# Angtian/VoGE

Hardware: AMD Instinct MI355X
Metric: forward+backward frames/sec at 512^2, 50k Gaussians; ray-trace HBM GB/s vs peak (higher is better)
Workload: dtype f32; 1 GPU; cfg3_50k_512: 50000 random Gaussians (scalar sigmas), 512x512, K=40, max_point_per_bin=-1, fwd+bwd (grads to verts, sigmas, colors); launch=hip graph replay, 4 consecutive steps per graph launch, parallelism=1 gpu

## Files before the change

include/voge_hip.h:

```cpp
#ifndef VOGE_HIP_H
#define VOGE_HIP_H

#include <stddef.h>
#include <stdint.h>

#ifdef __cplusplus
extern "C" {
#endif

#define VOGE_ABI_VERSION 7

#define VOGE_ERR_BAD_ARG (-1)
#define VOGE_ERR_WORKSPACE (-2)
#define VOGE_ERR_K_TOO_LARGE (-3)

#define VOGE_MAX_K 256

typedef void *voge_stream_t;

int voge_abi_version(void);

const char *voge_error_string(int code);

size_t voge_trace_workspace_bytes(int B, int N, int H, int W);
// ... 19 lines not shown
                   const float *g_dsd, int P, long nrows, int W, int K, void *workspace,
                   size_t workspace_bytes, float *g_ray, float *g_mus, float *g_isg,
                   voge_stream_t stream);

size_t voge_trace_bwd_workspace_bytes(int P);

int voge_trace_topk_fwd_iso(const float *mus, const float *a, const float *rays,
                            const float *cam_fwd, const float *cones, int B, int N, int H, int W, int K,
                            float thr_act, void *workspace, size_t workspace_bytes,
                            int32_t *idx, float *len, float *act, float *dsd, int32_t *cnt,
                            voge_stream_t stream);
int voge_trace_bwd_iso(const float *mus, const float *a, const float *rays, const int32_t *idx,
                       const int32_t *cnt, const float *g_len, const float *g_act, const float *g_dsd,
                       int P, long nrows, int W, int K, void *workspace, size_t workspace_bytes,
                       float *g_ray, float *g_mus, float *g_a, voge_stream_t stream);
size_t voge_trace_bwd_iso_workspace_bytes(int P);

int voge_trace_topk_fwd_iso_view(const float *verts, const float *sigmas, const float *origin, int shared,
                                 int sigma_mode, const float *rays, const float *cam_fwd, const float *cones,
                                 int B, int N, int H, int W, int K, float thr_act, void *workspace,
                                 size_t workspace_bytes, int32_t *idx, float *len, float *act, float *dsd,
                                 int32_t *cnt, voge_stream_t stream);
int voge_trace_bwd_iso_view(const float *verts, const float *sigmas, const float *origin, int shared,
                            int sigma_mode, const float *rays, const int32_t *idx, const int32_t *cnt,
                            const float *g_len, const float *g_act, const float *g_dsd, int B, int N, long nrows,
                            int W, int K, void *workspace, size_t workspace_bytes, float *g_ray,
                            float *g_verts, float *g_sigmas, voge_stream_t stream);

int voge_bin_gaussians(const float *points, const int64_t *cloud_to_packed_first_idx,
                       const int64_t *num_points_per_cloud, int B, int P, int H, int W, const float *radius,
                       int bin_size, int max_points_per_bin, int32_t *bin_elems, voge_stream_t stream);

int voge_trace_lean_fwd(const float *mus, const float *isigmas, const float *rays, const float *cam_fwd,
                        const float *cones, int B, int N, int H, int W, int K, float thr_act, void *workspace,
                        size_t workspace_bytes, int32_t *idx, float *len, int32_t *cnt, float *records,
                        voge_stream_t stream);
int voge_fragments_fwd(const float *mus, const float *isigmas, const float *rays, const float *cam_fwd,
                       const float *cones, int B, int N, int H, int W, int K, float thr_act, float occ,
                       void *workspace, size_t workspace_bytes, int32_t *idx, float *len, float *act, float *dsd,
                       int32_t *cnt, float *weight, int64_t *valid_num, voge_stream_t stream);
int voge_fragments_fwd_iso(const float *mus, const float *a, const float *rays, const float *cam_fwd,
                           const float *cones, int B, int N, int H, int W, int K, float thr_act, float occ,
                           void *workspace, size_t workspace_bytes, int32_t *idx, float *len, float *act,
                           float *dsd, int32_t *cnt, float *weight, int64_t *valid_num, float *records,
                           voge_stream_t stream);
int voge_fragments_fwd_iso_view(const float *verts, const float *sigmas, const float *origin, int shared,
                                int sigma_mode, const float *rays, const float *cam_fwd, const float *cones,
                                int B, int N, int H, int W, int K, float thr_act, float occ, void *workspace,
                                size_t workspace_bytes, int32_t *idx, float *len, float *act, float *dsd,
                                int32_t *cnt, float *weight, int64_t *valid_num, float *records, voge_stream_t stream);

size_t voge_fragment_bwd_workspace_bytes(int P);
int voge_fragment_act_dsd_iso(const float *records, const float *rays, const int32_t *idx, const float *len,
                              const int32_t *cnt, long npix, int K, int P, float *act, float *dsd, voge_stream_t stream);
int voge_composite_fwd_iso(const int32_t *idx, const int32_t *cnt, const float *len, const float *records,
                           const float *rays, float occ, long npix, int K, float *weight, int64_t *valid_num,
                           voge_stream_t stream);
int voge_composite_shade_fwd_iso(int32_t *idx, const int32_t *cnt, const float *len, const float *records,
                                 const float *rays, float occ, const float *colors, const float *bg, float thr,
                                 long npix, int K, int C, long Nattr, float *weight, int64_t *valid_num, float *rgb,
                                 float *img, float *wsum, voge_stream_t stream);
int voge_composite_fwd_rec(int32_t *idx, const int32_t *cnt, const float *len, const float *records, const float *rays,
                           float occ, long npix, int K, float *weight, int64_t *valid_num, float *act, float *dsd,
                           voge_stream_t stream);
int voge_composite_shade_fwd_rec(int32_t *idx, const int32_t *cnt, const float *len, const float *records,
                                 const float *rays, float occ, const float *colors, const float *bg, float thr,
                                 long npix, int K, int C, long Nattr, float *weight, int64_t *valid_num, float *rgb,
                                 float *img, float *wsum, float *act, float *dsd, voge_stream_t stream);
int voge_fragment_shade_bwd(const float *mus, const float *isigmas, const float *rays, const float *colors,
                            const int32_t *idx, const int32_t *cnt, const float *weight, const float *act,
                            const float *len, const float *dsd, const float *rgb, const float *wsum, const float *bg,
                            float thr, const float *g_img, long g_stride_pix, long g_stride_c, float occ, int P,
                            long nrows, int W, int K, int C, long Nattr, void *workspace, size_t workspace_bytes,
                            float *g_mus, float *g_isigmas, float *g_colors, voge_stream_t stream);
int voge_fragment_shade_bwd_iso(const float *records, const float *sigmas, int shared, int sigma_mode,
                                const float *rays, const float *colors, const int32_t *idx, const int32_t *cnt,
                                const float *weight, const float *act, const float *len, const float *dsd,
                                const float *rgb, const float *wsum, const float *bg, float thr,
                                const float *g_img, long g_stride_pix, long g_stride_c, float occ, int B, int N,
                                long nrows, int W, int K, int C, long Nattr, void *workspace, size_t workspace_bytes, float *g_verts,
                                float *g_sigmas, float *g_colors, voge_stream_t stream);

size_t voge_frame_bwd_acc_bytes(int P);
int voge_frame_trace_fwd_iso(const float *verts, const float *sigmas, int shared, int sigma_mode, const float *R,
                             const float *T, const float *focal, const float *pp, int row0, int stripe_h, int pitch,
                             int behind, int B, int N, int h, int W, int K, float thr_act, void *workspace,
                             size_t workspace_bytes, int32_t *idx, float *len, int32_t *cnt, float *records,
                             float *rays, float *origin, voge_stream_t stream);
int voge_frame_shade_fwd_iso(int32_t *idx, const int32_t *cnt, const float *len, const float *records,
                             const float *rays, float occ, const float *colors, const float *bg, float thr,
                             long npix, int K, int C, long Nattr, float *weight, int64_t *valid_num,
                             float *rgb, float *img, float *wsum, float *sil, void *bwd_acc, size_t bwd_acc_bytes,
                             voge_stream_t stream);
int voge_frame_shade_bwd_iso(const float *records, const float *sigmas, int shared, int sigma_mode,
                             const float *rays, const float *colors, const int32_t *idx, const int32_t *cnt,
                             const float *weight, const float *len, const float *rgb, const float *wsum,
                             const float *bg, float thr, const float *g_img, long g_stride_pix, long g_stride_c,
                             float occ, int B, int N, long nrows, int W, int K, int C, long Nattr, void *acc_zeroed,
                             size_t acc_bytes, float *g_verts, float *g_sigmas, float *g_colors, voge_stream_t stream);
int voge_frame_merge_bwd_iso(const float *records, const float *sigmas, int shared, int sigma_mode,
                             const float *rays, const float *attr, const int32_t *idx, const int32_t *cnt,
                             const float *weight, const float *len, const float *g_rgb, long g_stride_pix,
                             long g_stride_c, const float *g_wsum, const float *wsum_fwd, float occ, int B, int N, long nrows,
                             int W, int K, int C, long Nattr, void *acc_zeroed, size_t acc_bytes, float *g_verts,
                             float *g_sigmas, float *g_attr, voge_stream_t stream);

size_t voge_frame_bwd_gen_acc_bytes(int P);
int voge_frame_trace_fwd_gen(const float *verts, const float *sigmas, int shared_verts, int shared_sigmas, int kind,
                             const float *R, const float *T, const float *focal, const float *pp, int row0, int stripe_h,
                             int pitch, int behind, int B, int N, int h, int W, int K, float thr_act, void *workspace,
                             size_t workspace_bytes, int32_t *idx, float *len, int32_t *cnt, float *records, float *rays,
                             float *origin, voge_stream_t stream);
int voge_frame_shade_fwd_rec(int kind, int32_t *idx, const int32_t *cnt, const float *len, const float *records,
                             const float *rays, float occ, const float *colors, const float *bg, float thr,
                             long npix, int K, int C, long Nattr, float *weight, int64_t *valid_num,
                             float *rgb, float *img, float *wsum, float *sil, float *act, float *dsd, void *bwd_acc,
                             size_t bwd_acc_bytes, voge_stream_t stream);
int voge_frame_bwd_gen(int form, const float *records, int shared_verts, int shared_sigmas, int kind, const float *rays,
                       const float *attr, const int32_t *idx, const int32_t *cnt, const float *weight, const float *act,
                       const float *len, const float *dsd, const float *rgb, const float *wsum, const float *bg, float thr,
                       const float *g, long g_stride0, long g_stride1, const float *g_hitlen, float occ, int B, int N,
                       long nrows, int W, int K, int C, long Nattr, void *acc, size_t acc_bytes, int acc_is_zero,
                       float *g_verts, float *g_sigmas, float *g_attr, voge_stream_t stream);

int voge_frame_trace_fwd_ori(const float *verts, const float *scales, const float *quats, int shared_verts, int shared_sigmas,
                             int sigma_mode, const float *R, const float *T, const float *focal, const float *pp, int row0,
                             int stripe_h, int pitch, int behind, int B, int N, int h, int W, int K, float thr_act, void *workspace,
                             size_t workspace_bytes, int32_t *idx, float *len, int32_t *cnt, float *records, float *rays,
                             float *origin, voge_stream_t stream);
int voge_frame_bwd_ori(int form, const float *records, const float *scales, const float *quats, int shared_verts, int shared_sigmas,
                       int sigma_mode, const float *rays, const float *attr, const int32_t *idx, const int32_t *cnt,
                       const float *weight, const float *act, const float *len, const float *dsd, const float *rgb, const float *wsum,
                       const float *bg, float thr, const float *g, long g_stride0, long g_stride1, const float *g_hitlen, float occ,
                       int B, int N, long nrows, int W, int K, int C, long Nattr, void *acc, size_t acc_bytes, int acc_is_zero,
                       float *g_verts, float *g_scales, float *g_quats, float *g_attr, voge_stream_t stream);

int voge_fragment_merge_bwd(const float *mus, const float *isigmas, const float *rays, const float *attr,
                            const int32_t *idx, const int32_t *cnt, const float *weight, const float *act,
                            const float *len, const float *dsd, const float *g_rgb, long g_stride_pix,
                            long g_stride_c, const float *g_wsum, float occ, int P, long nrows, int W, int K, int C,
                            long Nattr, void *workspace, size_t workspace_bytes, float *g_mus, float *g_isigmas,
                            float *g_attr, voge_stream_t stream);
int voge_fragment_merge_bwd_iso(const float *records, const float *sigmas, int shared, int sigma_mode,
                                const float *rays, const float *attr, const int32_t *idx, const int32_t *cnt,
                                const float *weight, const float *act, const float *len, const float *dsd,
                                const float *g_rgb, long g_stride_pix, long g_stride_c, const float *g_wsum,
                                float occ, int B, int N, long nrows, int W, int K, int C, long Nattr,
                                void *workspace, size_t workspace_bytes, float *g_verts, float *g_sigmas,
                                float *g_attr, voge_stream_t stream);

int voge_fragment_bwd_iso(const float *records, const float *sigmas, int shared, int sigma_mode, const float *rays,
                          const int32_t *idx, const int32_t *cnt, const float *weight, const float *act,
                          const float *len, const float *dsd, const float *g_weight, long gw_stride_pix,
                          long gw_stride_k, const float *g_hitlen, float occ, int B, int N, long nrows, int W, int K,
                          void *workspace, size_t workspace_bytes, float *g_verts, float *g_sigmas,
                          voge_stream_t stream);
int voge_fragment_bwd(const float *mus, const float *isigmas, const float *rays, const int32_t *idx,
                      const int32_t *cnt, const float *weight, const float *act, const float *len,
                      const float *dsd, const float *g_weight, long gw_stride_pix, long gw_stride_k,
                      const float *g_hitlen, float occ, int P, long nrows, int W, int K, void *workspace,
                      size_t workspace_bytes, float *g_mus, float *g_isigmas, voge_stream_t stream);

int voge_composite_fwd(const int32_t *idx, const int32_t *cnt, const float *act, const float *len,
                       const float *dsd, float occ, long npix, int K, float *weight,
                       int64_t *valid_num, voge_stream_t stream);

// ... 91 lines not shown
```

voge_amd/_lib.py:

```python
import ctypes
import os

_HERE = os.path.dirname(os.path.abspath(__file__))
LIB_PATH = os.environ.get("VOGE_HIP_LIB") or os.path.join(_HERE, "libvoge_hip.so")
ABI_VERSION = 7
MAX_K = 256

_c_void_p = ctypes.c_void_p
_c_int = ctypes.c_int
_c_long = ctypes.c_long
_c_float = ctypes.c_float
_c_size_t = ctypes.c_size_t

SIGNATURES = {
    "voge_abi_version": (_c_int, []),
    "voge_error_string": (ctypes.c_char_p, [_c_int]),
    "voge_trace_workspace_bytes": (_c_size_t, [_c_int] * 4),
    "voge_trace_pool_usage": (_c_int, [_c_void_p, _c_size_t] + [_c_int] * 4 + [_c_void_p] * 2),
    "voge_trace_topk_fwd": (_c_int, [_c_void_p] * 5 + [_c_int] * 5 + [_c_float, _c_void_p, _c_size_t]
                            + [_c_void_p] * 6),
    "voge_trace_topk_list_fwd": (_c_int, [_c_void_p] * 4 + [_c_int] * 9 + [_c_float] + [_c_void_p] * 6),
    "voge_trace_bwd": (_c_int, [_c_void_p] * 8 + [_c_int, _c_long, _c_int, _c_int, _c_void_p, _c_size_t] + [_c_void_p] * 4),
    "voge_trace_bwd_workspace_bytes": (_c_size_t, [_c_int]),
    "voge_trace_topk_fwd_iso": (_c_int, [_c_void_p] * 5 + [_c_int] * 5 + [_c_float, _c_void_p, _c_size_t]
                                + [_c_void_p] * 6),
    "voge_trace_bwd_iso": (_c_int, [_c_void_p] * 8 + [_c_int, _c_long, _c_int, _c_int, _c_void_p, _c_size_t] + [_c_void_p] * 4),
    "voge_trace_bwd_iso_workspace_bytes": (_c_size_t, [_c_int]),
    "voge_trace_topk_fwd_iso_view": (_c_int, [_c_void_p] * 3 + [_c_int] * 2 + [_c_void_p] * 3 + [_c_int] * 5
                                     + [_c_float, _c_void_p, _c_size_t] + [_c_void_p] * 6),
    "voge_trace_bwd_iso_view": (_c_int, [_c_void_p] * 3 + [_c_int] * 2 + [_c_void_p] * 6
                                + [_c_int, _c_int, _c_long, _c_int, _c_int, _c_void_p, _c_size_t] + [_c_void_p] * 4),
    "voge_bin_gaussians": (_c_int, [_c_void_p] * 3 + [_c_int] * 4 + [_c_void_p] + [_c_int] * 2 + [_c_void_p] * 2),
    "voge_fragments_fwd": (_c_int, [_c_void_p] * 5 + [_c_int] * 5 + [_c_float, _c_float, _c_void_p, _c_size_t] + [_c_void_p] * 8),
    "voge_fragments_fwd_iso": (_c_int, [_c_void_p] * 5 + [_c_int] * 5 + [_c_float, _c_float, _c_void_p, _c_size_t] + [_c_void_p] * 9),
    "voge_fragments_fwd_iso_view": (_c_int, [_c_void_p] * 3 + [_c_int] * 2 + [_c_void_p] * 3 + [_c_int] * 5
                                    + [_c_float, _c_float, _c_void_p, _c_size_t] + [_c_void_p] * 9),
    "voge_frame_trace_fwd_iso": (_c_int, [_c_void_p] * 2 + [_c_int] * 2 + [_c_void_p] * 4 + [_c_int] * 9
                                 + [_c_float, _c_void_p, _c_size_t] + [_c_void_p] * 7),
    "voge_frame_shade_fwd_iso": (_c_int, [_c_void_p] * 5 + [_c_float, _c_void_p, _c_void_p, _c_float, _c_long, _c_int, _c_int, _c_long]
                                 + [_c_void_p] * 7 + [_c_size_t, _c_void_p]),
    "voge_frame_shade_bwd_iso": (_c_int, [_c_void_p] * 2 + [_c_int] * 2 + [_c_void_p] * 9 + [_c_float, _c_void_p, _c_long, _c_long, _c_float]
                                 + [_c_int, _c_int, _c_long, _c_int, _c_int, _c_int, _c_long, _c_void_p, _c_size_t] + [_c_void_p] * 4),
    "voge_frame_merge_bwd_iso": (_c_int, [_c_void_p] * 2 + [_c_int] * 2 + [_c_void_p] * 7 + [_c_long, _c_long, _c_void_p, _c_void_p, _c_float]
                                 + [_c_int, _c_int, _c_long, _c_int, _c_int, _c_int, _c_long, _c_void_p, _c_size_t] + [_c_void_p] * 4),
    "voge_frame_bwd_acc_bytes": (_c_size_t, [_c_int]),
    "voge_frame_bwd_gen_acc_bytes": (_c_size_t, [_c_int]),
    "voge_frame_trace_fwd_gen": (_c_int, [_c_void_p] * 2 + [_c_int] * 3 + [_c_void_p] * 4 + [_c_int] * 9
                                 + [_c_float, _c_void_p, _c_size_t] + [_c_void_p] * 7),
    "voge_frame_shade_fwd_rec": (_c_int, [_c_int] + [_c_void_p] * 5 + [_c_float, _c_void_p, _c_void_p, _c_float, _c_long, _c_int, _c_int, _c_long]
                                 + [_c_void_p] * 9 + [_c_size_t, _c_void_p]),
    "voge_frame_bwd_gen": (_c_int, [_c_int, _c_void_p] + [_c_int] * 3 + [_c_void_p] * 11 + [_c_float, _c_void_p, _c_long, _c_long, _c_void_p, _c_float]
                           + [_c_int, _c_int, _c_long, _c_int, _c_int, _c_int, _c_long, _c_void_p, _c_size_t, _c_int] + [_c_void_p] * 4),
    "voge_frame_trace_fwd_ori": (_c_int, [_c_void_p] * 3 + [_c_int] * 3 + [_c_void_p] * 4 + [_c_int] * 9
                                 + [_c_float, _c_void_p, _c_size_t] + [_c_void_p] * 7),
    "voge_frame_bwd_ori": (_c_int, [_c_int] + [_c_void_p] * 3 + [_c_int] * 3 + [_c_void_p] * 11 + [_c_float, _c_void_p, _c_long, _c_long, _c_void_p, _c_float]
                           + [_c_int, _c_int, _c_long, _c_int, _c_int, _c_int, _c_long, _c_void_p, _c_size_t, _c_int] + [_c_void_p] * 5),
    "voge_fragment_bwd_workspace_bytes": (_c_size_t, [_c_int]),
    "voge_fragment_act_dsd_iso": (_c_int, [_c_void_p] * 5 + [_c_long, _c_int, _c_int] + [_c_void_p] * 3),
    "voge_composite_shade_fwd_iso": (_c_int, [_c_void_p] * 5 + [_c_float, _c_void_p, _c_void_p, _c_float, _c_long, _c_int, _c_int, _c_long]
                                     + [_c_void_p] * 6),
    "voge_composite_shade_fwd_rec": (_c_int, [_c_void_p] * 5 + [_c_float, _c_void_p, _c_void_p, _c_float, _c_long, _c_int, _c_int, _c_long]
                                     + [_c_void_p] * 8),
    "voge_composite_fwd_rec": (_c_int, [_c_void_p] * 5 + [_c_float, _c_long, _c_int] + [_c_void_p] * 5),
    "voge_trace_lean_fwd": (_c_int, [_c_void_p] * 5 + [_c_int] * 5 + [_c_float, _c_void_p, _c_size_t] + [_c_void_p] * 5),
    "voge_fragment_merge_bwd": (_c_int, [_c_void_p] * 11 + [_c_long, _c_long, _c_void_p, _c_float, _c_int, _c_long, _c_int, _c_int, _c_int,
                                                             _c_long, _c_void_p, _c_size_t] + [_c_void_p] * 4),
    "voge_composite_fwd_iso": (_c_int, [_c_void_p] * 5 + [_c_float, _c_long, _c_int] + [_c_void_p] * 3),
    "voge_fragment_shade_bwd": (_c_int, [_c_void_p] * 13 + [_c_float, _c_void_p, _c_long, _c_long, _c_float]
                                + [_c_int, _c_long, _c_int, _c_int, _c_int, _c_long, _c_void_p, _c_size_t] + [_c_void_p] * 4),
    "voge_fragment_shade_bwd_iso": (_c_int, [_c_void_p] * 2 + [_c_int] * 2 + [_c_void_p] * 11 + [_c_float, _c_void_p, _c_long, _c_long, _c_float]
                                    + [_c_int, _c_int, _c_long, _c_int, _c_int, _c_int, _c_long, _c_void_p, _c_size_t] + [_c_void_p] * 4),
    "voge_fragment_merge_bwd_iso": (_c_int, [_c_void_p] * 2 + [_c_int] * 2 + [_c_void_p] * 9 + [_c_long, _c_long, _c_void_p, _c_float]
                                    + [_c_int, _c_int, _c_long, _c_int, _c_int, _c_int, _c_long, _c_void_p, _c_size_t] + [_c_void_p] * 4),
    "voge_fragment_bwd_iso": (_c_int, [_c_void_p] * 2 + [_c_int] * 2 + [_c_void_p] * 8 + [_c_long, _c_long, _c_void_p, _c_float]
                              + [_c_int, _c_int, _c_long, _c_int, _c_int, _c_void_p, _c_size_t] + [_c_void_p] * 3),
    "voge_fragment_bwd": (_c_int, [_c_void_p] * 10 + [_c_long, _c_long, _c_void_p, _c_float]
                          + [_c_int, _c_long, _c_int, _c_int, _c_void_p, _c_size_t] + [_c_void_p] * 3),
    "voge_composite_fwd": (_c_int, [_c_void_p] * 5 + [_c_float, _c_long, _c_int] + [_c_void_p] * 3),
    "voge_composite_bwd": (_c_int, [_c_void_p] * 6 + [_c_float, _c_long, _c_int] + [_c_void_p] * 4),
    "voge_merge_fwd": (_c_int, [_c_void_p] * 4 + [_c_long, _c_int, _c_int, _c_long, _c_int] + [_c_void_p] * 2),
    "voge_merge_bwd": (_c_int, [_c_void_p] * 5 + [_c_long, _c_int, _c_int, _c_int, _c_long] + [_c_void_p] * 3),
    "voge_blend_fwd": (_c_int, [_c_void_p] * 3 + [_c_float, _c_long, _c_int, _c_int] + [_c_void_p] * 3),
    "voge_shade_fwd": (_c_int, [_c_void_p] * 5 + [_c_float, _c_long, _c_int, _c_int, _c_long, _c_int] + [_c_void_p] * 5),
    "voge_shade_bwd": (_c_int, [_c_void_p] * 7 + [_c_float, _c_void_p, _c_long, _c_int, _c_int, _c_int, _c_long] + [_c_void_p] * 3),
    "voge_rays_fwd": (_c_int, [_c_void_p] * 4 + [_c_int] * 4 + [_c_void_p] * 4),
    "voge_rays_striped_fwd": (_c_int, [_c_void_p] * 4 + [_c_int] * 6 + [_c_void_p] * 4),
    "voge_rays_striped_bwd": (_c_int, [_c_void_p] * 6 + [_c_int] * 6 + [_c_void_p] * 6),
    "voge_cones_floats": (_c_size_t, [_c_int] * 3),
    "voge_ray_cones": (_c_int, [_c_void_p, _c_int, _c_int, _c_int, _c_void_p, _c_void_p]),
    "voge_general_preamble_fwd": (_c_int, [_c_void_p] * 3 + [_c_int] * 5 + [_c_void_p] * 3),
    "voge_general_preamble_bwd": (_c_int, [_c_void_p] * 2 + [_c_int] * 5 + [_c_void_p] * 3),
    "voge_rays_bwd": (_c_int, [_c_void_p] * 6 + [_c_int] * 4 + [_c_void_p] * 6),
    "voge_ray_dense_fwd": (_c_int, [_c_void_p] * 3 + [_c_int, _c_long] + [_c_void_p] * 4),
    "voge_ray_dense_bwd": (_c_int, [_c_void_p] * 6 + [_c_int, _c_long] + [_c_void_p] * 4),
    "voge_find_nearest_k": (_c_int, [_c_void_p] * 3 + [_c_float, _c_int, _c_int, _c_long] + [_c_void_p] * 5),
    "voge_find_nearest_k_bwd": (_c_int, [_c_void_p] * 4 + [_c_int, _c_int, _c_long] + [_c_void_p] * 4),
    "voge_scatter_max": (_c_int, [_c_void_p] * 2 + [_c_long, _c_long] + [_c_void_p] * 2),
    "voge_silhouette_fwd": (_c_int, [_c_void_p, _c_long, _c_int] + [_c_void_p] * 3),
    "voge_silhouette_bwd": (_c_int, [_c_void_p] * 2 + [_c_long] + [_c_void_p] * 2),
    "voge_blend_bwd": (_c_int, [_c_void_p] * 3 + [_c_float, _c_void_p, _c_long, _c_int, _c_int] + [_c_void_p] * 3),
    "voge_blend_bg_fwd": (_c_int, [_c_void_p] * 3 + [_c_long] * 4 + [_c_float] + [_c_int] * 4 + [_c_void_p] * 2),
    "voge_blend_bg_bwd": (_c_int, [_c_void_p] * 3 + [_c_long] * 4 + [_c_float, _c_void_p, _c_long, _c_long] + [_c_int] * 4
                          + [_c_void_p] * 3 + [_c_long] * 4 + [_c_void_p, _c_size_t, _c_void_p]),
    "voge_blend_bg_bwd_workspace_bytes": (_c_size_t, [_c_int] * 4),
}

_lib = None


class VogeHipError(RuntimeError):
    """Raised when libvoge_hip.so is missing or one of its entry points returns non-zero
    (the reference raises RuntimeError through AT_CUDA_CHECK, ray_trace_voge.cu:278)."""


def load():
    global _lib
    if _lib is not None:
        return _lib
    if not os.path.exists(LIB_PATH):
# ... 51 lines not shown
```

voge_amd/csrc/trace_bin.h:

```cpp
#pragma once
#include <type_traits>

#include "voge_common.h"

namespace voge {

constexpr int kST0 = 128;
constexpr int kCh = kST0 / kST;
constexpr int kBinThreads = 1024;
constexpr int kParts = 16;
constexpr int kSegCap = 512;
constexpr int kTileCap = 2048;
constexpr int kTilesPerBin = (kST / 8) * (kST / 8);
constexpr int kRankMaxBins = 4096;
static_assert(kCh * kCh == kBinThreads / 64, "one wave per super-tile of a region / per sweep tile of a super-tile");

__device__ __forceinline__ float depth_key(const float4 c, const Cone &k) {
  const float nm = sqrtf(fmaf(c.z, c.z, fmaf(c.y, c.y, c.x * c.x)));
  const float R = c.w;
  if (!(R < 3e38f) || !(nm < 3e38f)) return -INFINITY;
  float kappa = -nm;
  if (k.ok && k.cs >= 0.5f && nm > 4.0f * R) {
    const float p = fmaf(c.z, k.az, fmaf(c.y, k.ay, c.x * k.ax));
    if (p > 0.0f) kappa = nm;
  }
  return kappa;
}

__device__ __forceinline__ float4 iso_cull_record(const float mx, const float my, const float mz, const float a,
                                                  const float thr_act) {
  float reach = INFINITY;
  if (a > 0.0f && a < 3e38f) {
    const float nm = __builtin_amdgcn_sqrtf(fmaf(mz, mz, fmaf(my, my, mx * mx)));
    const float r = __builtin_amdgcn_sqrtf(fmaxf(thr_act, 0.0f) * __builtin_amdgcn_rcpf(a * (1.0f - 4e-6f))) * (1.0f + 2e-5f) + 2e-5f * nm + 1e-30f;
    reach = r;
    if (!(reach >= 0.0f)) reach = INFINITY;
    if (reach < 3e38f) reach = __uint_as_float((__float_as_uint(reach) + 1u) & ~1u);
  }
  return make_float4(mx, my, mz, reach);
}

#ifdef VOGE_BIN_TIMES
__device__ unsigned long long g_bin_times[2][1024 * 8];
__device__ unsigned long long g_bin_wave[1024 * 16 * 4];
#define BIN_WTS(k) \
  if ((threadIdx.x & 63) == 0 && blockIdx.y == 0 && blockIdx.x < 1024) g_bin_wave[(blockIdx.x * 16 + (threadIdx.x >> 6)) * 4 + (k)] = wall_clock64()
#define BIN_TS(which, k) \
  if (threadIdx.x == 0 && blockIdx.y == 0 && blockIdx.x < 1024) g_bin_times[which][8 * blockIdx.x + (k)] = wall_clock64()
#else
#define BIN_TS(which, k)
#define BIN_WTS(k)
#endif

constexpr int kRoundChunks = 4;
constexpr int kRoundCap = kRoundChunks * kBinThreads;

constexpr int kExtMul = 3;
constexpr int kExtChunk = 1024;
constexpr int kExtChunks = 16;
__host__ __device__ inline int slice_cap(const int N) {
  return ((N + kParts * kBinThreads - 1) / (kParts * kBinThreads)) * kBinThreads;
}
struct BinALds {
  int arena_top;
  int extc[kCh * kCh][kExtChunks];
  int extn[kCh * kCh];
  float4 srec[kRoundCap];
  int sid[kRoundCap];
  ConeRec child[kCh * kCh];
  ConeRec region;
  ConeRec rowc[kCh];
  int use_rows;
  int cnt0[kRoundChunks][16];
  int base[kCh * kCh];
  int nS;
};

struct BinARaw {
  float4 v;
};
struct BinAView {
  float ox, oy, oz;
  float fx, fy, fz;
  bool has_f;
};
template <bool ISO_PREP>
__device__ __forceinline__ BinAView binA_view(const int b, const float *__restrict__ cam_fwd, const IsoView view,
                                              const CamView &cam = no_camera(), const CamK *ck = nullptr) {
  BinAView V;
  V.ox = V.oy = V.oz = 0.f; V.fx = V.fy = V.fz = 0.f; V.has_f = false;
  if (ISO_PREP) {
    if (view.origin != nullptr) { const float *o = view.origin + 3 * b; V.ox = o[0]; V.oy = o[1]; V.oz = o[2]; }
    if (cam_fwd != nullptr) { const float *f = cam_fwd + 3 * b; V.fx = f[0]; V.fy = f[1]; V.fz = f[2]; V.has_f = true; }
    if (cam.R != nullptr) {
      cam_origin(*ck, cam.T + 3 * b, V.ox, V.oy, V.oz);
      if (cam.behind) { const float *r = cam.R + 9 * b; V.fx = r[2]; V.fy = r[5]; V.fz = r[8]; V.has_f = true; }
    }
  }
  return V;
}
template <bool ISO_PREP>
__device__ __forceinline__ BinARaw binA_fetch(const int g, const int b, const int N, const float4 *__restrict__ cull,
                                              const float *__restrict__ mus, const float *__restrict__ isg, const IsoView view) {
  BinARaw r;
  r.v = make_float4(0.f, 0.f, 0.f, 0.f);
  if (N <= 0) return r;
  const int gc = max(g, 0);
  if (!ISO_PREP) { r.v = cull[(size_t)b * N + gc]; return r; }
  const size_t src = view.shared ? (size_t)gc : (size_t)b * N + gc;
  r.v = make_float4(mus[3 * src + 0], mus[3 * src + 1], mus[3 * src + 2], isg[src]);
  return r;
}
template <bool ISO_PREP>
__device__ __forceinline__ float4 binA_derive(const BinARaw r, const bool valid, const BinAView &V, const float thr_act,
                                              const IsoView view, float &a_out) {
  a_out = 0.f;
  if (!valid) return make_float4(0.f, 0.f, 0.f, -1.f);
  if (!ISO_PREP) return r.v;
  float mx = r.v.x, my = r.v.y, mz = r.v.z;
  if (view.origin != nullptr || view.cam_origin) { mx -= V.ox; my -= V.oy; mz -= V.oz; }
  const float a = iso_view_a(r.v.w, view.mode);
  a_out = a;
  float4 c = iso_cull_record(mx, my, mz, a, thr_act);
  if (V.has_f && fmaf(mz, V.fz, fmaf(my, V.fy, mx * V.fx)) < 0.0f) c.w = -1.0f;
  return c;
}

__host__ __device__ inline bool deal_interleaved(const int N) { return N < kParts * kBinThreads; }
__device__ __forceinline__ int slice_of(const int g, const int N) {
  return deal_interleaved(N) ? g % kParts : (g / kBinThreads) % kParts;
}

template <bool ISO_PREP>
__global__ void __launch_bounds__(kBinThreads)
binA_kernel(const ConeRec *__restrict__ cones , const int nstx, const int nsty, const int nst0x,
            const float *__restrict__ mus, const float *__restrict__ isg, const float *__restrict__ cam_fwd, const int N,
            const float thr_act, const IsoView view, float4 *__restrict__ cull, float4 *__restrict__ ms,
            int *__restrict__ seg_count , int32_t *__restrict__ seg_id ,
            float4 *__restrict__ seg_rec ,
            unsigned long long *__restrict__ pool_top ,
            int *__restrict__ seg_ext ,
            int32_t *__restrict__ ext_id , const int ext_arena,
            const CamView cam ) {
  __shared__ BinALds L;
  const int tid = threadIdx.x, lane = tid & 63, wave = tid >> 6;
  const int region = blockIdx.x / kParts, part = blockIdx.x - region * kParts;
  const int b = blockIdx.y;
  if (blockIdx.x == 0 && blockIdx.y == 0 && tid == 0) *pool_top = 0ull;
  const int rx = region % nst0x, ry = region / nst0x;
  const int nst = nstx * nsty;
  if (tid < kCh * kCh) { L.base[tid] = 0; L.extn[tid] = 0; }
  if (tid == 0) L.arena_top = 0;
  int32_t *const arena = ext_id + ((size_t)(b * (int)(gridDim.x / kParts) + region) * kParts + part) * (size_t)ext_arena;
  int ext_have = 0;
  BIN_TS(0, 0);
  const bool interleaved = deal_interleaved(N);
  const int nchunks = interleaved ? kParts * ((N + kParts * kBinThreads - 1) / (kParts * kBinThreads))
                                  : (N + kBinThreads - 1) / kBinThreads;
  const bool writes_records = ISO_PREP && region == 0;
  float4 c[kRoundChunks];
  float av[kRoundChunks];
  int gq[kRoundChunks];
  CamK ck;
  if (cam.R != nullptr) ck = cam_load(cam, b);
  const BinAView V = binA_view<ISO_PREP>(b, cam_fwd, view, cam, &ck);
  if (cam.R != nullptr && cam.origin_out != nullptr && blockIdx.x == 0 && tid == 0) {
    cam.origin_out[3 * b] = V.ox; cam.origin_out[3 * b + 1] = V.oy; cam.origin_out[3 * b + 2] = V.oz;
  }
  BinARaw raw[kRoundChunks];
  auto fetch_round = [&](const int j0) {
#pragma unroll
    for (int q = 0; q < kRoundChunks; ++q) {
      const int j = j0 + q * kParts;
      const int g = interleaved ? ((j / kParts) * kBinThreads + tid) * kParts + part : j * kBinThreads + tid;
      gq[q] = (j < nchunks && g < N) ? g : -1;
      raw[q] = binA_fetch<ISO_PREP>(gq[q], b, N, cull, mus, isg, view);
    }
  };
  auto derive_round = [&]() {
#pragma unroll
    for (int q = 0; q < kRoundChunks; ++q) c[q] = binA_derive<ISO_PREP>(raw[q], gq[q] >= 0, V, thr_act, view, av[q]);
  };
  auto load_round = [&](const int j0) { fetch_round(j0); derive_round(); };
  fetch_round(part);
  if (wave == 0) {
    const int cc = lane & (kCh * kCh - 1);
    const int cx = rx * kCh + (cc & (kCh - 1)), cy = ry * kCh + cc / kCh;
    ConeRec r = {0.f, 0.f, 1.f, 1.f, 0.f, -1.f, 0.f, 0.f};
    const bool region_rect = cam.R != nullptr && cam.h <= cam.stripe_h;
    if (cam.R != nullptr) {
      const bool reg = region_rect && lane == kCh * kCh;
      const int j0 = reg ? rx * kCh * kST : cx * kST, i0 = reg ? ry * kCh * kST : cy * kST, ext = reg ? kCh * kST : kST;
      if ((cx < nstx && cy < nsty) || reg) r = cam_rect_cone(ck, cam, j0, j0 + ext - 1, i0, i0 + ext - 1);
    } else if (cx < nstx && cy < nsty) {
      r = cones[cone_super_at(b, nst, cy * nstx + cx)];
    }
    if (lane < kCh * kCh) L.child[lane] = r;
    if (region_rect) {
      if (lane == kCh * kCh) L.region = r;
      if (lane == 0) L.use_rows = 0;
    } else {
    const bool present = lane < kCh * kCh && r.ok >= 0.f;
    const float sx = wave_sum_dpp(present ? r.ax : 0.f), sy = wave_sum_dpp(present ? r.ay : 0.f), sz = wave_sum_dpp(present ? r.az : 0.f);
    const float npres = wave_sum_dpp(present ? 1.f : 0.f);
    bool ok = __all(!present || r.ok > 0.f);
    const float n = sqrtf(fmaf(sz, sz, fmaf(sy, sy, sx * sx)));
    const float ax = sx / n, ay = sy / n, az = sz / n;
    auto child_extrema = [&](const float ax_, const float ay_, const float az_, float &smax_, float &cmin_, bool &ok_) {
      smax_ = 0.f; cmin_ = 1.f;
      if (present) {
        const float ca = fmaf(r.az, az_, fmaf(r.ay, ay_, r.ax * ax_));
        const float qx = fmaf(-ca, ax_, r.ax), qy = fmaf(-ca, ay_, r.ay), qz = fmaf(-ca, az_, r.az);
        const float sa = sqrtf(fmaf(qz, qz, fmaf(qy, qy, qx * qx))) * (1.0f + 1e-6f) + 1e-7f;
        const float cl = fminf(ca, 1.0f) - 1e-7f;
        if (!(cl > 0.0f)) ok_ = false;
        cmin_ = fmaf(cl, r.cs, -sa * r.sn);
        smax_ = fmaf(fminf(ca + 1e-7f, 1.0f), r.sn, sa);
      }
    };
    float smax, cmin;
    child_extrema(ax, ay, az, smax, cmin, ok);
    ok = __all(ok);
    smax = wave_max(smax); cmin = wave_min(cmin);
    const Cone cn = cone_finish(ax, ay, az, n / fmaxf(npres, 1.f), smax, cmin, ok);
    if (lane == 0) L.region = ConeRec{cn.ax, cn.ay, cn.az, cn.cs, cn.sn, cn.ok ? 1.f : 0.f, 0.f, 0.f};
    const float widest_child = wave_max(present ? (r.ok > 0.f ? r.sn : 2.0f) : 0.f);
    if (lane == 0) L.use_rows = 0;
    if (__builtin_expect((!cn.ok || cn.sn > 8.0f * widest_child) && N < (1 << 27), 0)) {
      auto quad_sum = [](float v) { v += VOGE_DPP(v, 0xB1); v += VOGE_DPP(v, 0x4E); return v; };
      auto quad_max = [](float v) { v = fmaxf(v, VOGE_DPP(v, 0xB1)); v = fmaxf(v, VOGE_DPP(v, 0x4E)); return v; };
      auto quad_min = [](float v) { v = fminf(v, VOGE_DPP(v, 0xB1)); v = fminf(v, VOGE_DPP(v, 0x4E)); return v; };
      static_assert(kCh == 4, "a row of super-tiles is a DPP quad");
      const float qsx = quad_sum(present ? r.ax : 0.f), qsy = quad_sum(present ? r.ay : 0.f), qsz = quad_sum(present ? r.az : 0.f);
      const float qn = quad_sum(present ? 1.f : 0.f);
      const float nn = sqrtf(fmaf(qsz, qsz, fmaf(qsy, qsy, qsx * qsx)));
      const float rax = qsx / nn, ray = qsy / nn, raz = qsz / nn;
      float rs, rc;
      bool rok = !present || r.ok > 0.f;
      child_extrema(rax, ray, raz, rs, rc, rok);
      rs = quad_max(rs); rc = quad_min(rc);
      const float okf = quad_min(rok ? 1.f : 0.f);
      const Cone rcn = cone_finish(rax, ray, raz, nn / fmaxf(qn, 1.f), rs, rc, okf != 0.f);
      if (lane < kCh * kCh && (lane & 3) == 0) L.rowc[lane >> 2] = ConeRec{rcn.ax, rcn.ay, rcn.az, rcn.cs, rcn.sn, qn > 0.f ? (rcn.ok ? 1.f : 0.f) : -1.f, 0.f, 0.f};
      const float widest_row = wave_max((lane < kCh * kCh && qn > 0.f) ? (rcn.ok ? rcn.sn : 2.0f) : 0.f);
      if (lane == 0) L.use_rows = (!cn.ok || cn.sn > 1.6f * widest_row) ? 1 : 0;
    }
    }
  }
  BIN_TS(0, 6);
  derive_round();
// ... 807 lines not shown
```

voge_amd/csrc/trace_fwd.hip:

```cpp
#include "voge_common.h"

namespace voge {

__device__ inline double lambda_min_sym3(double a00, double a11, double a22, double a01,
                                         double a02, double a12) {
  const double p1 = a01 * a01 + a02 * a02 + a12 * a12;
  if (p1 == 0.0) return fmin(a00, fmin(a11, a22));
  const double q = (a00 + a11 + a22) / 3.0;
  const double b00 = a00 - q, b11 = a11 - q, b22 = a22 - q;
  const double p2 = b00 * b00 + b11 * b11 + b22 * b22 + 2.0 * p1;
  const double p = sqrt(p2 / 6.0);
  const double ip = 1.0 / p;
  const double c00 = b00 * ip, c11 = b11 * ip, c22 = b22 * ip;
  const double c01 = a01 * ip, c02 = a02 * ip, c12 = a12 * ip;
  double r = 0.5 * (c00 * (c11 * c22 - c12 * c12) - c01 * (c01 * c22 - c12 * c02) +
                    c02 * (c01 * c12 - c11 * c02));
  r = fmin(1.0, fmax(-1.0, r));
  const double phi = acos(r) / 3.0;
  return q + 2.0 * p * cos(phi + 2.0943951023931953);
}

__device__ __forceinline__ void prep_one(const int g, const float *__restrict__ mus, const float *__restrict__ isg,
                                         const float *__restrict__ cam_fwd, const int N, const float thr_act,
                                         const int iso_in, float4 *__restrict__ cull, float4 *__restrict__ evr,
// ... 1333 lines not shown
extern "C" int voge_trace_topk_fwd_iso(const float *mus, const float *a, const float *rays,
                                       const float *cam_fwd, const float *cones, int B, int N, int H, int W, int K,
                                       float thr_act, void *workspace, size_t workspace_bytes,
                                       int32_t *idx, float *len, float *act, float *dsd, int32_t *cnt,
                                       voge_stream_t stream) {
  return trace_topk_fwd_impl(1, IsoView{nullptr, 0, 0}, mus, a, rays, cam_fwd, cones, B, N, H, W, K, thr_act, workspace,
                             workspace_bytes, idx, len, act, dsd, cnt, stream);
}

extern "C" int voge_trace_topk_list_fwd(const float *mus, const float *isigmas, const float *rays,
                                        const int32_t *bin_points, int B, int P, int H, int W, int K,
                                        int BH, int BW, int M, int bin_size, float thr_act,
                                        int32_t *idx, float *len, float *act, float *dsd, int32_t *cnt,
                                        voge_stream_t stream) {
  if (B < 0 || P < 0 || H < 0 || W < 0 || K <= 0 || BH <= 0 || BW <= 0 || M < 0 || bin_size <= 0)
    return VOGE_ERR_BAD_ARG;
  if (K > VOGE_MAX_K) return VOGE_ERR_K_TOO_LARGE;
  if ((size_t)B * H * W == 0) return 0;
  if (!rays || !idx || !len || !act || !dsd || (M > 0 && !bin_points)) return VOGE_ERR_BAD_ARG;
  if (P > 0 && (!mus || !isigmas)) return VOGE_ERR_BAD_ARG;
  const size_t lds = sizeof(uint64_t) * (size_t)K * 64;
  {
    static DynLdsCache cache;
    const int rc = ensure_dynamic_lds(reinterpret_cast<const void *>(trace_list_fwd_kernel), lds, cache);
    if (rc) return rc;
  }
  dim3 grid(((W + 7) / 8) * ((H + 7) / 8), B);
  hipLaunchKernelGGL(trace_list_fwd_kernel, grid, dim3(64), lds, (hipStream_t)stream, mus, isigmas, rays,
                     bin_points, P, H, W, K, BH, BW, M, bin_size, thr_act, idx, len, act, dsd, cnt);
  return launch_status();
}

extern "C" int voge_trace_topk_fwd_iso_view(const float *verts, const float *sigmas, const float *origin, int shared,
                                            int sigma_mode, const float *rays, const float *cam_fwd, const float *cones,
                                            int B, int N, int H, int W, int K, float thr_act, void *workspace,
                                            size_t workspace_bytes, int32_t *idx, float *len, float *act, float *dsd,
                                            int32_t *cnt, voge_stream_t stream) {
  if (sigma_mode < 0 || sigma_mode > 2) return VOGE_ERR_BAD_ARG;
  return trace_topk_fwd_impl(1, IsoView{origin, shared ? 1 : 0, sigma_mode}, verts, sigmas, rays, cam_fwd, cones, B, N, H, W, K,
                             thr_act, workspace, workspace_bytes, idx, len, act, dsd, cnt, stream);
}

extern "C" int voge_trace_lean_fwd(const float *mus, const float *isigmas, const float *rays, const float *cam_fwd,
                                   const float *cones, int B, int N, int H, int W, int K, float thr_act, void *workspace,
                                   size_t workspace_bytes, int32_t *idx, float *len, int32_t *cnt, float *records,
                                   voge_stream_t stream) {
  if (!cnt || !records) return VOGE_ERR_BAD_ARG;
  return trace_topk_fwd_impl(0, IsoView{nullptr, 0, 0}, mus, isigmas, rays, cam_fwd, cones, B, N, H, W, K, thr_act, workspace,
                             workspace_bytes, idx, len, nullptr, nullptr, cnt, stream, 1.0f, nullptr, nullptr, records);
}

extern "C" int voge_fragments_fwd(const float *mus, const float *isigmas, const float *rays, const float *cam_fwd,
                                  const float *cones, int B, int N, int H, int W, int K, float thr_act, float occ,
                                  void *workspace, size_t workspace_bytes, int32_t *idx, float *len, float *act, float *dsd,
                                  int32_t *cnt, float *weight, int64_t *valid_num, voge_stream_t stream) {
  if (!weight || !valid_num || !cnt) return VOGE_ERR_BAD_ARG;
  return trace_topk_fwd_impl(0, IsoView{nullptr, 0, 0}, mus, isigmas, rays, cam_fwd, cones, B, N, H, W, K, thr_act, workspace,
                             workspace_bytes, idx, len, act, dsd, cnt, stream, occ, weight, valid_num);
}

extern "C" int voge_fragments_fwd_iso(const float *mus, const float *a, const float *rays, const float *cam_fwd,
                                      const float *cones, int B, int N, int H, int W, int K, float thr_act, float occ,
                                      void *workspace, size_t workspace_bytes, int32_t *idx, float *len, float *act,
                                      float *dsd, int32_t *cnt, float *weight, int64_t *valid_num, float *records,
                                      voge_stream_t stream) {
  if (!cnt || (weight == nullptr) != (valid_num == nullptr) || (!weight && (!records || act || dsd))) return VOGE_ERR_BAD_ARG;
  return trace_topk_fwd_impl(1, IsoView{nullptr, 0, 0}, mus, a, rays, cam_fwd, cones, B, N, H, W, K, thr_act, workspace,
                             workspace_bytes, idx, len, act, dsd, cnt, stream, occ, weight, valid_num, records);
}

extern "C" int voge_fragments_fwd_iso_view(const float *verts, const float *sigmas, const float *origin, int shared,
                                           int sigma_mode, const float *rays, const float *cam_fwd, const float *cones,
                                           int B, int N, int H, int W, int K, float thr_act, float occ, void *workspace,
                                           size_t workspace_bytes, int32_t *idx, float *len, float *act, float *dsd,
                                           int32_t *cnt, float *weight, int64_t *valid_num, float *records,
                                           voge_stream_t stream) {
  if (sigma_mode < 0 || sigma_mode > 2 || !cnt || (weight == nullptr) != (valid_num == nullptr) ||
      (!weight && (!records || act || dsd)))
    return VOGE_ERR_BAD_ARG;
  return trace_topk_fwd_impl(1, IsoView{origin, shared ? 1 : 0, sigma_mode}, verts, sigmas, rays, cam_fwd, cones, B, N, H, W, K,
                             thr_act, workspace, workspace_bytes, idx, len, act, dsd, cnt, stream, occ, weight, valid_num, records);
}

extern "C" int voge_frame_trace_fwd_iso(const float *verts, const float *sigmas, int shared, int sigma_mode, const float *R,
                                        const float *T, const float *focal, const float *pp, int row0, int stripe_h, int pitch,
                                        int behind, int B, int N, int h, int W, int K, float thr_act, void *workspace,
                                        size_t workspace_bytes, int32_t *idx, float *len, int32_t *cnt, float *records,
                                        float *rays, float *origin, voge_stream_t stream) {
  if (sigma_mode < 0 || sigma_mode > 2 || !cnt || !records || !R || !T || !focal || !pp || stripe_h <= 0 || pitch < 0)
    return VOGE_ERR_BAD_ARG;
  if ((size_t)B * h * W > 0 && !rays) return VOGE_ERR_BAD_ARG;
  const CamView cam{R, T, focal, pp, row0, stripe_h, pitch, h, W, behind ? 1 : 0, origin, rays};
  return trace_topk_fwd_impl(1, IsoView{nullptr, shared ? 1 : 0, sigma_mode}, verts, sigmas, nullptr, nullptr, nullptr, B, N, h, W, K,
                             thr_act, workspace, workspace_bytes, idx, len, nullptr, nullptr, cnt, stream, 1.0f, nullptr, nullptr, records,
                             cam);
}

extern "C" int voge_frame_trace_fwd_gen(const float *verts, const float *sigmas, int shared_verts, int shared_sigmas, int kind,
                                        const float *R, const float *T, const float *focal, const float *pp, int row0, int stripe_h,
                                        int pitch, int behind, int B, int N, int h, int W, int K, float thr_act, void *workspace,
                                        size_t workspace_bytes, int32_t *idx, float *len, int32_t *cnt, float *records, float *rays,
                                        float *origin, voge_stream_t stream) {
  if ((kind != 1 && kind != 2) || !cnt || !records || !R || !T || !focal || !pp || stripe_h <= 0 || pitch < 0) return VOGE_ERR_BAD_ARG;
  if ((size_t)B * h * W > 0 && !rays) return VOGE_ERR_BAD_ARG;
  const CamView cam{R, T, focal, pp, row0, stripe_h, pitch, h, W, behind ? 1 : 0, origin, rays};
  IsoView view{nullptr, shared_verts ? 1 : 0, 0};
  view.gen_kind = kind; view.sigma_shared = shared_sigmas ? 1 : 0;
  return trace_topk_fwd_impl(0, view, verts, sigmas, nullptr, nullptr, nullptr, B, N, h, W, K, thr_act, workspace, workspace_bytes, idx, len,
                             nullptr, nullptr, cnt, stream, 1.0f, nullptr, nullptr, records, cam);
}

extern "C" int voge_frame_trace_fwd_ori(const float *verts, const float *scales, const float *quats, int shared_verts,
                                        int shared_sigmas, int sigma_mode, const float *R, const float *T, const float *focal,
                                        const float *pp, int row0, int stripe_h, int pitch, int behind, int B, int N, int h, int W,
                                        int K, float thr_act, void *workspace, size_t workspace_bytes, int32_t *idx, float *len,
                                        int32_t *cnt, float *records, float *rays, float *origin, voge_stream_t stream) {
  if ((sigma_mode != 1 && sigma_mode != 2) || !cnt || !records || !R || !T || !focal || !pp || stripe_h <= 0 || pitch < 0) return VOGE_ERR_BAD_ARG;
  if ((size_t)B * h * W > 0 && !rays) return VOGE_ERR_BAD_ARG;
  if (N > 0 && (!quats || (reinterpret_cast<uintptr_t>(quats) & 15) != 0)) return VOGE_ERR_BAD_ARG;
  const CamView cam{R, T, focal, pp, row0, stripe_h, pitch, h, W, behind ? 1 : 0, origin, rays};
  IsoView view{nullptr, shared_verts ? 1 : 0, 0};
  view.gen_kind = 3; view.sigma_shared = shared_sigmas ? 1 : 0; view.quats = quats; view.ori_mode = sigma_mode;
  return trace_topk_fwd_impl(0, view, verts, scales, nullptr, nullptr, nullptr, B, N, h, W, K, thr_act, workspace, workspace_bytes, idx, len,
                             nullptr, nullptr, cnt, stream, 1.0f, nullptr, nullptr, records, cam);
}
```

voge_amd/csrc/voge_common.h:

```cpp
#pragma once
#include <hip/hip_runtime.h>
#include <stdint.h>

#include <atomic>

#include "voge_hip.h"

#define VOGE_WAVE 64

#define VOGE_SENT_LEN 1e10f
#define VOGE_SENT_ACT 1e10f

namespace voge {

struct EvalRec {
  float s00, s11, s22, s01, s02, s12;
  float bx, by, bz;
  float kx, ky, kz;
};
static_assert(sizeof(EvalRec) == 48, "EvalRec must be 3 x float4");

__device__ __forceinline__ float fast_div(const float a, const float b) { return a * __builtin_amdgcn_rcpf(b); }

constexpr uint32_t kIsoFlag = 0x7fc0a150u;
// ... 255 lines not shown
    }
    keys[(unsigned)pos * (unsigned)stride] = key;
    if (full) {
      tail = top;
      worst = top;
    } else if (++cnt == K) {
      worst = tail;
    }
  }
}

__device__ __forceinline__ float wave_sum(float v) {
#pragma unroll
  for (int o = 32; o > 0; o >>= 1) v += __shfl_xor(v, o, 64);
  return v;
}
typedef float voge_v4f __attribute__((ext_vector_type(4)));
typedef int voge_v4i __attribute__((ext_vector_type(4)));
template <bool NT>
__device__ __forceinline__ void st16f(float *p, const float a, const float b, const float c, const float d) {
  const voge_v4f v = {a, b, c, d};
  if (NT) __builtin_nontemporal_store(v, reinterpret_cast<voge_v4f *>(p)); else *reinterpret_cast<voge_v4f *>(p) = v;
}
__device__ __forceinline__ __amdgpu_buffer_rsrc_t out_rsrc(void *base, const unsigned bytes) {
  return __builtin_amdgcn_make_buffer_rsrc(base, 0, (int)bytes, 0x00020000);
}
__device__ __forceinline__ void st16f_wt(const __amdgpu_buffer_rsrc_t r, const unsigned byte_off, const float a, const float b,
                                         const float c, const float d) {
  const voge_v4f v = {a, b, c, d};
  __builtin_amdgcn_raw_buffer_store_b128(v, r, (int)byte_off, 0, 16 );
}
__device__ __forceinline__ void st16i_wt(const __amdgpu_buffer_rsrc_t r, const unsigned byte_off, const int a, const int b,
                                         const int c, const int d) {
  const voge_v4i v = {a, b, c, d};
  __builtin_amdgcn_raw_buffer_store_b128(v, r, (int)byte_off, 0, 16 );
}
template <bool NT>
__device__ __forceinline__ void st16i(int32_t *p, const int a, const int b, const int c, const int d) {
  const voge_v4i v = {a, b, c, d};
  if (NT) __builtin_nontemporal_store(v, reinterpret_cast<voge_v4i *>(p)); else *reinterpret_cast<voge_v4i *>(p) = v;
}
#define VOGE_DPP(v, ctrl) __int_as_float(__builtin_amdgcn_update_dpp(0, __float_as_int(v), ctrl, 0xF, 0xF, true))
#define VOGE_LANE(v, l) __int_as_float(__builtin_amdgcn_readlane(__float_as_int(v), l))
__device__ __forceinline__ float wave_max(float v) {
  v = fmaxf(v, VOGE_DPP(v, 0xB1));
  v = fmaxf(v, VOGE_DPP(v, 0x4E));
  v = fmaxf(v, VOGE_DPP(v, 0x141));
  v = fmaxf(v, VOGE_DPP(v, 0x140));
  return fmaxf(fmaxf(VOGE_LANE(v, 0), VOGE_LANE(v, 16)), fmaxf(VOGE_LANE(v, 32), VOGE_LANE(v, 48)));
}
__device__ __forceinline__ float wave_min(float v) {
  v = fminf(v, VOGE_DPP(v, 0xB1));
  v = fminf(v, VOGE_DPP(v, 0x4E));
  v = fminf(v, VOGE_DPP(v, 0x141));
  v = fminf(v, VOGE_DPP(v, 0x140));
  return fminf(fminf(VOGE_LANE(v, 0), VOGE_LANE(v, 16)), fminf(VOGE_LANE(v, 32), VOGE_LANE(v, 48)));
}
__device__ __forceinline__ int wave_incl_scan_i32(int v) {
  v += __builtin_amdgcn_update_dpp(0, v, 0x111, 0xF, 0xF, true);
  v += __builtin_amdgcn_update_dpp(0, v, 0x112, 0xF, 0xF, true);
  v += __builtin_amdgcn_update_dpp(0, v, 0x114, 0xF, 0xF, true);
  v += __builtin_amdgcn_update_dpp(0, v, 0x118, 0xF, 0xF, true);
  v += __builtin_amdgcn_update_dpp(0, v, 0x142, 0xA, 0xF, false);
  v += __builtin_amdgcn_update_dpp(0, v, 0x143, 0xC, 0xF, false);
  return v;
}
__device__ __forceinline__ float wave_sum_dpp(float v) {
  v += VOGE_DPP(v, 0xB1);
  v += VOGE_DPP(v, 0x4E);
  v += VOGE_DPP(v, 0x141);
  v += VOGE_DPP(v, 0x140);
  return (VOGE_LANE(v, 0) + VOGE_LANE(v, 16)) + (VOGE_LANE(v, 32) + VOGE_LANE(v, 48));
}

struct Cone {
  float ax, ay, az, cs, sn;
  bool ok;
};

__device__ __forceinline__ bool cone_keep(const float4 c, const Cone &k) {
  if (c.w < 0.0f) return false;
  const float p = fmaf(c.z, k.az, fmaf(c.y, k.ay, c.x * k.ax));
  const float rx = fmaf(-p, k.ax, c.x), ry = fmaf(-p, k.ay, c.y), rz = fmaf(-p, k.az, c.z);
  const float q = sqrtf(fmaf(rz, rz, fmaf(ry, ry, rx * rx)));
  const float gap = fmaf(q, k.cs, -fabsf(p) * k.sn);
  return !k.ok || !(gap > c.w);
}

constexpr int kST = 32;

struct RayDir {
  float ux, uy, uz;
  bool ok;
  bool unit;
};
__device__ __forceinline__ RayDir ray_dir(const float dx, const float dy, const float dz) {
  RayDir r;
  const float dn2 = fmaf(dz, dz, fmaf(dy, dy, dx * dx));
  const float inv = 1.0f / sqrtf(dn2);
  r.ok = (dn2 > 0.0f) && (inv < 3e38f) && (inv == inv);
  r.unit = fabsf(dn2 - 1.0f) < 1e-4f;
  r.ux = dx * inv; r.uy = dy * inv; r.uz = dz * inv;
  return r;
}
__device__ __forceinline__ void cone_partial(const RayDir &u, const float ax, const float ay, const float az,
                                             float &smax, float &cmin) {
  const float cl = fmaf(u.uz, az, fmaf(u.uy, ay, u.ux * ax));
  const float rx = fmaf(-cl, ax, u.ux), ry = fmaf(-cl, ay, u.uy), rz = fmaf(-cl, az, u.uz);
  const float sl = sqrtf(fmaf(rz, rz, fmaf(ry, ry, rx * rx)));
  smax = fmaxf(smax, u.ok ? sl : 2.0f);
  cmin = fminf(cmin, u.ok ? cl : -1.0f);
}
__device__ __forceinline__ Cone cone_finish(const float ax, const float ay, const float az, const float n,
                                            const float smax, const float cmin, const bool all_ok) {
  Cone c;
  c.ax = ax; c.ay = ay; c.az = az;
  c.sn = smax * (1.0f + 1e-5f) + 1e-7f;
  c.cs = cmin - 1e-6f;
  c.ok = all_ok && (n > 1e-3f) && (cmin > 0.05f) && (c.sn == c.sn);
  return c;
}

struct ConeRec {
  float ax, ay, az, cs, sn, ok, pad0, pad1;
};
__device__ __forceinline__ Cone load_cone(const ConeRec &r) {
  Cone c;
  c.ax = r.ax; c.ay = r.ay; c.az = r.az; c.cs = r.cs; c.sn = r.sn; c.ok = r.ok > 0.f;
  return c;
}

struct Mat3 {
  float m[9];
};
__device__ __forceinline__ Mat3 inv3(const float *R) {
  Mat3 o;
  const float a = R[0], b = R[1], c = R[2], d = R[3], e = R[4], f = R[5], g = R[6], h = R[7], i = R[8];
  const float A = e * i - f * h, B = -(d * i - f * g), C = d * h - e * g;
  const float det = a * A + b * B + c * C;
  const float id = 1.0f / det;
  o.m[0] = A * id;               o.m[1] = -(b * i - c * h) * id;  o.m[2] = (b * f - c * e) * id;
  o.m[3] = B * id;               o.m[4] = (a * i - c * g) * id;   o.m[5] = -(a * f - c * d) * id;
  o.m[6] = C * id;               o.m[7] = -(a * h - b * g) * id;  o.m[8] = (a * e - b * d) * id;
  return o;
}
struct CamView {
  const float *R, *T, *focal, *pp;
  int row0, stripe_h, pitch;
  int h, W;
  int behind;
  float *origin_out;
  float *rays_out;
};
__host__ __device__ inline CamView no_camera() { return CamView{nullptr, nullptr, nullptr, nullptr, 0, 1, 0, 0, 0, 0, nullptr, nullptr}; }
struct CamK {
  Mat3 Ri;
  float ifx, ify, px, py;
};
__device__ __forceinline__ CamK cam_load(const CamView &c, const int b) {
  CamK k;
  k.Ri = inv3(c.R + 9 * b);
  k.ifx = 1.0f / c.focal[2 * b]; k.ify = 1.0f / c.focal[2 * b + 1];
  k.px = c.pp[2 * b]; k.py = c.pp[2 * b + 1];
  return k;
}
__device__ __forceinline__ int cam_irow(const CamView &c, const int i) {
  if (i < c.stripe_h) return c.row0 + i;
// ... 478 lines not shown
```

Measured before the change: 4214 frames/s.

## Add camera-cone precompute kernel and use hardware sqrt in cone culling

Adds a new exported kernel that precomputes per-tile, per-quad, per-super-tile and per-region cone records from camera parameters. It also switches cone-culling and depth-key square roots to the raw hardware sqrt builtin, dropping the precise-sqrt correction sequence, and makes the binning kernel compute the camera origin when not in iso-prep mode. The new cone entry point is not wired into the existing frame path, so only the sqrt change and origin tweak affect the default pipeline. The hardware sqrt is less exact, which can shift culling decisions at boundaries.

```diff
diff --git a/include/voge_hip.h b/include/voge_hip.h
--- a/include/voge_hip.h
+++ b/include/voge_hip.h
@@ -125,6 +125,9 @@
                                 float *g_sigmas, float *g_colors, voge_stream_t stream);
 
 size_t voge_frame_bwd_acc_bytes(int P);
+int voge_camera_cones(const float *R, const float *T, const float *focal, const float *pp, int row0, int stripe_h, int pitch,
+                      int B, int h, int W, float *hier, float *regions, voge_stream_t stream);
+
 int voge_frame_trace_fwd_iso(const float *verts, const float *sigmas, int shared, int sigma_mode, const float *R,
                              const float *T, const float *focal, const float *pp, int row0, int stripe_h, int pitch,
                              int behind, int B, int N, int h, int W, int K, float thr_act, void *workspace,
diff --git a/voge_amd/_lib.py b/voge_amd/_lib.py
--- a/voge_amd/_lib.py
+++ b/voge_amd/_lib.py
@@ -35,6 +35,7 @@
     "voge_fragments_fwd_iso": (_c_int, [_c_void_p] * 5 + [_c_int] * 5 + [_c_float, _c_float, _c_void_p, _c_size_t] + [_c_void_p] * 9),
     "voge_fragments_fwd_iso_view": (_c_int, [_c_void_p] * 3 + [_c_int] * 2 + [_c_void_p] * 3 + [_c_int] * 5
                                     + [_c_float, _c_float, _c_void_p, _c_size_t] + [_c_void_p] * 9),
+    "voge_camera_cones": (_c_int, [_c_void_p] * 4 + [_c_int] * 6 + [_c_void_p] * 3),
     "voge_frame_trace_fwd_iso": (_c_int, [_c_void_p] * 2 + [_c_int] * 2 + [_c_void_p] * 4 + [_c_int] * 9
                                  + [_c_float, _c_void_p, _c_size_t] + [_c_void_p] * 7),
     "voge_frame_shade_fwd_iso": (_c_int, [_c_void_p] * 5 + [_c_float, _c_void_p, _c_void_p, _c_float, _c_long, _c_int, _c_int, _c_long]
diff --git a/voge_amd/csrc/trace_bin.h b/voge_amd/csrc/trace_bin.h
--- a/voge_amd/csrc/trace_bin.h
+++ b/voge_amd/csrc/trace_bin.h
@@ -16,7 +16,7 @@
 static_assert(kCh * kCh == kBinThreads / 64, "one wave per super-tile of a region / per sweep tile of a super-tile");
 
 __device__ __forceinline__ float depth_key(const float4 c, const Cone &k) {
-  const float nm = sqrtf(fmaf(c.z, c.z, fmaf(c.y, c.y, c.x * c.x)));
+  const float nm = __builtin_amdgcn_sqrtf(fmaf(c.z, c.z, fmaf(c.y, c.y, c.x * c.x)));
   const float R = c.w;
   if (!(R < 3e38f) || !(nm < 3e38f)) return -INFINITY;
   float kappa = -nm;
@@ -165,7 +165,9 @@
   if (cam.R != nullptr) ck = cam_load(cam, b);
   const BinAView V = binA_view<ISO_PREP>(b, cam_fwd, view, cam, &ck);
   if (cam.R != nullptr && cam.origin_out != nullptr && blockIdx.x == 0 && tid == 0) {
-    cam.origin_out[3 * b] = V.ox; cam.origin_out[3 * b + 1] = V.oy; cam.origin_out[3 * b + 2] = V.oz;
+    float ox = V.ox, oy = V.oy, oz = V.oz;
+    if (!ISO_PREP) cam_origin(ck, cam.T + 3 * b, ox, oy, oz);
+    cam.origin_out[3 * b] = ox; cam.origin_out[3 * b + 1] = oy; cam.origin_out[3 * b + 2] = oz;
   }
   BinARaw raw[kRoundChunks];
   auto fetch_round = [&](const int j0) {
diff --git a/voge_amd/csrc/trace_fwd.hip b/voge_amd/csrc/trace_fwd.hip
--- a/voge_amd/csrc/trace_fwd.hip
+++ b/voge_amd/csrc/trace_fwd.hip
@@ -1439,6 +1439,38 @@
                              thr_act, workspace, workspace_bytes, idx, len, act, dsd, cnt, stream, occ, weight, valid_num, records);
 }
 
+namespace voge {
+__global__ void __launch_bounds__(kQT)
+camera_cones_kernel(const CamView cam, const int nstx, const int nsty, const int nst0x, const int nst0y,
+                    ConeRec *__restrict__ hier , ConeRec *__restrict__ regions ) {
+  const int tid = threadIdx.x, wave = tid >> 6, b = blockIdx.y;
+  const int binl = blockIdx.x >> 2, qq = blockIdx.x & 3;
+  const int stx = binl % nstx, sty = binl / nstx;
+  const size_t nst = (size_t)nstx * nsty;
+  const CamK ck = cam_load(cam, b);
+  const int tx = stx * (kST / 8) + (qq & 1) * 2 + (wave & 1), ty = sty * (kST / 8) + (qq >> 1) * 2 + (wave >> 1);
+  ConeRec tcr, qcr;
+  cam_two_cones(ck, cam, tx * 8, ty * 8, 8, stx * kST + (qq & 1) * kQuad, sty * kST + (qq >> 1) * kQuad, kQuad, tcr, qcr);
+  if ((tid & 63) == 0) hier[cone_tile_at(b, nst, binl, ((qq >> 1) * 2 + (wave >> 1)) * 4 + (qq & 1) * 2 + (wave & 1))] = tcr;
+  if (tid == 0) hier[cone_quad_at(b, nst, binl, qq)] = qcr;
+  if (tid == 0 && qq == 0) hier[cone_super_at(b, nst, binl)] = cam_rect_cone(ck, cam, stx * kST, stx * kST + kST - 1, sty * kST, sty * kST + kST - 1);
+  if (tid == 0 && qq == 1 && binl < nst0x * nst0y) {
+    const int rx = binl % nst0x, ry = binl / nst0x;
+    regions[(size_t)b * nst0x * nst0y + binl] = cam_rect_cone(ck, cam, rx * kST0, rx * kST0 + kST0 - 1, ry * kST0, ry * kST0 + kST0 - 1);
+  }
+}
+}
+
+extern "C" int voge_camera_cones(const float *R, const float *T, const float *focal, const float *pp, int row0, int stripe_h, int pitch,
+                                 int B, int h, int W, float *hier, float *regions, voge_stream_t stream) {
+  if (!R || !T || !focal || !pp || !hier || !regions || stripe_h <= 0 || pitch < 0 || B <= 0 || h <= 0 || W <= 0) return VOGE_ERR_BAD_ARG;
+  const CamView cam{R, T, focal, pp, row0, stripe_h, pitch, h, W, 0, nullptr, nullptr};
+  const int nstx = (W + kST - 1) / kST, nsty = (h + kST - 1) / kST, nst0x = (W + kST0 - 1) / kST0, nst0y = (h + kST0 - 1) / kST0;
+  hipLaunchKernelGGL(camera_cones_kernel, dim3(nstx * nsty * 4, B), dim3(kQT), 0, (hipStream_t)stream, cam, nstx, nsty, nst0x, nst0y,
+                     reinterpret_cast<ConeRec *>(hier), reinterpret_cast<ConeRec *>(regions));
+  return launch_status();
+}
+
 extern "C" int voge_frame_trace_fwd_iso(const float *verts, const float *sigmas, int shared, int sigma_mode, const float *R,
                                         const float *T, const float *focal, const float *pp, int row0, int stripe_h, int pitch,
                                         int behind, int B, int N, int h, int W, int K, float thr_act, void *workspace,
diff --git a/voge_amd/csrc/voge_common.h b/voge_amd/csrc/voge_common.h
--- a/voge_amd/csrc/voge_common.h
+++ b/voge_amd/csrc/voge_common.h
@@ -361,7 +361,7 @@
   if (c.w < 0.0f) return false;
   const float p = fmaf(c.z, k.az, fmaf(c.y, k.ay, c.x * k.ax));
   const float rx = fmaf(-p, k.ax, c.x), ry = fmaf(-p, k.ay, c.y), rz = fmaf(-p, k.az, c.z);
-  const float q = sqrtf(fmaf(rz, rz, fmaf(ry, ry, rx * rx)));
+  const float q = __builtin_amdgcn_sqrtf(fmaf(rz, rz, fmaf(ry, ry, rx * rx)));
   const float gap = fmaf(q, k.cs, -fabsf(p) * k.sn);
   return !k.ok || !(gap > c.w);
 }
```

After: 4258 frames/s, median of 6. +1.1%, better.
